# input-output-hk/plutus-halo2-verifier-gen

Measured on AMD Instinct MI355X. Metric: halo2_proofs_verified_per_sec, higher is better.
Workload: dtype u32

## Files before the change

### plutus_halo2_verifier_gen_amd/csrc/bls_consts.h

```cpp
#pragma once
#include <stdint.h>
#define H2V_DEVCONST static constexpr __device__ uint32_t
H2V_DEVCONST FP_MOD[12] = {0xffffaaabu, 0xb9feffffu, 0xb153ffffu, 0x1eabfffeu, 0xf6b0f624u, 0x6730d2a0u, 0xf38512bfu, 0x64774b84u, 0x434bacd7u, 0x4b1ba7b6u, 0x397fe69au, 0x1a0111eau};
static constexpr uint32_t FP_N0 = 0xfffcfffdu;
H2V_DEVCONST FP_ONE[12] = {0x0347fcb8u, 0x19d80000u, 0x6d2002b1u, 0x12e00cdeu, 0xa2090c72u, 0x37669f83u, 0xda0f73e0u, 0x09b09b42u, 0x8f1297bbu, 0xa7c515d9u, 0xfcfa012cu, 0x0577a659u};
H2V_DEVCONST FP_R2[12] = {0x510370edu, 0x626d1c34u, 0xc53e243du, 0xd65aec45u, 0x3317d3b1u, 0x4f36a009u, 0x5d74088bu, 0x8c10ea72u, 0x75865d11u, 0xd507320au, 0xa759fd5cu, 0x0c8d4cc8u};
H2V_DEVCONST FP_MOD28[14] = {0xfffaaabu, 0xfefffffu, 0x3ffffb9u, 0xfffeb15u, 0x6241eabu, 0xa0f6b0fu, 0xf6730d2u, 0xf38512bu, 0x4774b84u, 0x4bacd76u, 0xba7b643u, 0xe69a4b1u, 0x1ea397fu, 0x001a011u};
static constexpr uint32_t FP_N0_28 = 0xffcfffdu;
static constexpr uint32_t FP_FOLD_M = 0x9d83u;
H2V_DEVCONST FP_ONE28[14] = {0x347fcb8u, 0xd800000u, 0x2b119u, 0xcde6d2u, 0xc7212e0u, 0x83a2090u, 0x37669fu, 0xda0f73eu, 0x9b09b42u, 0x1297bb0u, 0x515d98fu, 0x12ca7cu, 0x659fcfau, 0x577au};
H2V_DEVCONST FP_C23P28[14] = {0xcda8c09u, 0x8faaaaau, 0x15720a4u, 0x893d93u, 0xfad6c24u, 0x8d68ebau, 0x54754b0u, 0x8d36a8du, 0x7f2d603u, 0xd0496f2u, 0x7467875u, 0xa2fbde3u, 0xf8a1126u, 0xc501u};
H2V_DEVCONST FP_C23N28[14] = {0x3251ea2u, 0x6f55555u, 0x2a8df15u, 0xf76ad82u, 0x676b287u, 0x138dc54u, 0xa1fdc22u, 0x664e69eu, 0xc847581u, 0x7b63683u, 0x4613dcdu, 0x439e6ceu, 0x2602859u, 0xdb0fu};
H2V_DEVCONST F28_KP[5][14] = {{0x0u, 0x0u, 0x0u, 0x0u, 0x0u, 0x0u, 0x0u, 0x0u, 0x0u, 0x0u, 0x0u, 0x0u, 0x0u, 0x0u}, {0xfffaaabu, 0xfefffffu, 0x3ffffb9u, 0xfffeb15u, 0x6241eabu, 0xa0f6b0fu, 0xf6730d2u, 0xf38512bu, 0x4774b84u, 0x4bacd76u, 0xba7b643u, 0xe69a4b1u, 0x1ea397fu, 0x1a011u}, {0xfff5556u, 0xfdfffffu, 0x7ffff73u, 0xfffd62au, 0xc483d57u, 0x41ed61eu, 0xece61a5u, 0xe70a257u, 0x8ee9709u, 0x9759aecu, 0x74f6c86u, 0xcd34963u, 0x3d472ffu, 0x34022u}, {0xfff0001u, 0xfcfffffu, 0xbffff2du, 0xfffc13fu, 0x26c5c03u, 0xe2e412eu, 0xe359277u, 0xda8f383u, 0xd65e28eu, 0xe306862u, 0x2f722c9u, 0xb3cee15u, 0x5beac7fu, 0x4e033u}, {0xffeaaacu, 0xfbfffffu, 0xffffee7u, 0xfffac54u, 0x8907aafu, 0x83dac3du, 0xd9cc34au, 0xce144afu, 0x1dd2e13u, 0x2eb35d9u, 0xe9ed90du, 0x9a692c6u, 0x7a8e5ffu, 0x68044u}};
H2V_DEVCONST F28_BIAS_3_1[14] = {0x2fff0001u, 0x2fcffffdu, 0x2bffff2bu, 0x2fffc13du, 0x226c5c01u, 0x2e2e412cu, 0x2e359275u, 0x2da8f381u, 0x2d65e28cu, 0x2e306860u, 0x22f722c7u, 0x2b3cee13u, 0x25beac7du, 0x4e031u};
H2V_DEVCONST F28_BIAS_5_2[14] = {0x3ffe5557u, 0x3faffffcu, 0x33fffe9eu, 0x3fff9767u, 0x3eb49958u, 0x324d1749u, 0x3d03f41au, 0x3c1995d8u, 0x36547995u, 0x37a6034cu, 0x3a468f4du, 0x38103775u, 0x39931f7cu, 0x82052u};
H2V_DEVCONST F28_BIAS_6_1[14] = {0x2ffe0002u, 0x2f9ffffdu, 0x27fffe59u, 0x2fff827du, 0x24d8b805u, 0x2c5c825au, 0x2c6b24edu, 0x2b51e705u, 0x2acbc51bu, 0x2c60d0c3u, 0x25ee4591u, 0x2679dc28u, 0x2b7d58fdu, 0x9c064u};
H2V_DEVCONST F28_BIAS_7_1[14] = {0x2ffdaaadu, 0x2f8ffffdu, 0x2bfffe13u, 0x2fff6d92u, 0x2afcd6b1u, 0x266bed69u, 0x2bd255c0u, 0x2a8a3831u, 0x2f4310a0u, 0x211b9e39u, 0x2195fbd5u, 0x24e380dau, 0x2d67927du, 0xb6075u};
H2V_DEVCONST F28_BIAS_9_4[14] = {0x5ffd0003u, 0x5f6ffffau, 0x53fffd84u, 0x5fff43bau, 0x57451406u, 0x5a8ac385u, 0x5aa0b762u, 0x58fada86u, 0x5831a7a7u, 0x5a913923u, 0x58e56858u, 0x51b6ca3au, 0x513c057au, 0xea095u};
H2V_DEVCONST F28_BIAS_11_1[14] = {0x2ffc5559u, 0x2f4ffffdu, 0x2bfffcfbu, 0x2fff19e7u, 0x238d5161u, 0x2ea999a7u, 0x296f190au, 0x276b7ce1u, 0x21203eb4u, 0x2406d413u, 0x2034d4e2u, 0x2e8a13a1u, 0x2510787cu, 0x11e0bau};
H2V_DEVCONST F28_BIAS_13_2[14] = {0x3ffbaaafu, 0x3f2ffffcu, 0x33fffc6eu, 0x3ffef011u, 0x3fd58eb8u, 0x32c86fc4u, 0x383d7aafu, 0x35dc1f38u, 0x3a0ed5bdu, 0x3d7c6efeu, 0x37844167u, 0x3b5d5d03u, 0x38e4eb7bu, 0x1520dbu};
H2V_DEVCONST F28_BIAS_17_8[14] = {0x9ffa555bu, 0x9eeffff6u, 0x93fffb50u, 0x9ffe9c60u, 0x98660962u, 0x9b061bfcu, 0x95da3df3u, 0x92bd63e2u, 0x9bec03cbu, 0x9067a4d1u, 0x96231a6fu, 0x9503efc4u, 0x908dd175u, 0x1ba11au};
H2V_DEVCONST F28_BIAS_20_1[14] = {0x2ff9555cu, 0x2ebffffdu, 0x2ffffa85u, 0x2ffe5da6u, 0x2ad2656du, 0x29345d31u, 0x240fd072u, 0x2066576du, 0x2951e661u, 0x2e980d3bu, 0x291a3d3fu, 0x2040dde0u, 0x264c7dfcu, 0x208154u};
H2V_DEVCONST F28_BIAS_21_1[14] = {0x2ff90007u, 0x2eaffffdu, 0x23fffa3fu, 0x2ffe48bcu, 0x20f68419u, 0x2343c841u, 0x23770145u, 0x2f9ea899u, 0x2dc931e5u, 0x2352dab1u, 0x24c1f383u, 0x2eaa8292u, 0x2836b77bu, 0x222165u};
H2V_DEVCONST F28_BIAS_29_2[14] = {0x3ff6555fu, 0x3e2ffffcu, 0x33fff80eu, 0x3ffda165u, 0x32177978u, 0x33bf20bbu, 0x3eb087d9u, 0x396131f7u, 0x31838e0cu, 0x39294663u, 0x31ffa59cu, 0x31f7a81fu, 0x3788837au, 0x2f21edu};
H2V_DEVCONST F28_BIAS_32_1[14] = {0x2ff55560u, 0x2dfffffdu, 0x2ffff73du, 0x2ffd62a5u, 0x2483d57du, 0x21ed61eau, 0x2ce61a52u, 0x270a257cu, 0x2ee9709cu, 0x2759aec6u, 0x24f6c867u, 0x2d349635u, 0x2d472ffau, 0x340221u};
H2V_DEVCONST FP_MOD30[13] = {0x3fffaaabu, 0x27fbffffu, 0x153ffffbu, 0x2affffacu, 0x30f6241eu, 0x34a83dau, 0x112bf673u, 0x12e13ce1u, 0x2cd76477u, 0x1ed90d2eu, 0x29a4b1bau, 0x3a8e5ff9u, 0x1a0111u};
static constexpr uint32_t FP_MINV30 = 0x30003u;
H2V_DEVCONST FP_R3[12] = {0xd1f7b890u, 0x22294cc4u, 0x56c9f3afu, 0xc0ccb5bau, 0xd975ccb5u, 0x89a8c5c0u, 0x6c968b4cu, 0x922672eau, 0xa691de8cu, 0x7c835652u, 0xbbb98497u, 0x141ab424u};
H2V_DEVCONST FR_MOD30[9] = {0x1u, 0x3ffffffcu, 0x3fe5bfefu, 0x2f6900bfu, 0x21d80553u, 0x27602026u, 0x17d48333u, 0x29d4ca67u, 0x73edu};
static constexpr uint32_t FR_MINV30 = 0x1u;
H2V_DEVCONST FP_B[12] = {0x0d1ff2e0u, 0x67600000u, 0xb4800ac4u, 0x4b803379u, 0x882431c8u, 0xdd9a7e0eu, 0x683dcf80u, 0x26c26d0bu, 0x3c4a5eecu, 0x9f145766u, 0xf3e804b2u, 0x15de9967u};
H2V_DEVCONST FP_TWO224[12] = {0x883cb548u, 0x5e8f53dbu, 0x0373eaf8u, 0xb9b546d2u, 0x1904502cu, 0x51b9fef6u, 0xe94c8520u, 0x8388341au, 0x58c0fea4u, 0x2865518au, 0x2cc4653du, 0x0a82ce35u};
H2V_DEVCONST FP_HALF_PLAIN[12] = {0xffffd555u, 0xdcff7fffu, 0x58a9ffffu, 0x0f55ffffu, 0x7b587b12u, 0xb3986950u, 0x79c2895fu, 0xb23ba5c2u, 0x21a5d66bu, 0x258dd3dbu, 0x1cbff34du, 0x0d0088f5u};
H2V_DEVCONST FP_SQRT_EXP[12] = {0xffffeaabu, 0xee7fbfffu, 0xac54ffffu, 0x07aaffffu, 0x3dac3d89u, 0xd9cc34a8u, 0x3ce144afu, 0xd91dd2e1u, 0x90d2eb35u, 0x92c6e9edu, 0x8e5ff9a6u, 0x0680447au};
#define FP_SQRT_CHAIN_LEN 79
static constexpr __device__ uint8_t FP_SQRT_CHAIN[79][2] = {{4, 6}, {9, 0}, {4, 0}, {7, 7}, {4, 2}, {6, 3}, {6, 5}, {4, 7}, {4, 7}, {6, 6}, {6, 6}, {6, 4}, {3, 1}, {7, 6}, {4, 6}, {6, 7}, {5, 6}, {4, 4}, {8, 6}, {6, 5}, {3, 2}, {3, 1}, {6, 6}, {4, 3}, {3, 1}, {3, 0}, {6, 3}, {4, 3}, {5, 4}, {4, 3}, {8, 4}, {3, 3}, {5, 3}, {7, 2}, {7, 4}, {5, 5}, {4, 7}, {3, 1}, {5, 3}, {4, 1}, {8, 6}, {5, 2}, {2, 0}, {9, 7}, {5, 6}, {3, 1}, {8, 7}, {3, 1}, {7, 4}, {9, 7}, {4, 2}, {5, 5}, {4, 7}, {4, 7}, {4, 7}, {3, 3}, {5, 5}, {6, 2}, {5, 4}, {4, 7}, {4, 7}, {4, 7}, {4, 7}, {4, 6}, {2, 1}, {6, 7}, {4, 7}, {5, 7}, {4, 7}, {4, 7}, {4, 7}, {4, 7}, {4, 7}, {4, 7}, {4, 7}, {3, 2}, {4, 2}, {4, 2}, {3, 1}};
H2V_DEVCONST FP_BETA[12] = {0x8a75929au, 0x9d681b79u, 0x2bf22a3eu, 0xbb45abc0u, 0xe6e7e4e5u, 0x81411755u, 0x6d04f1b4u, 0xcae3387du, 0x4b54acb0u, 0x8b50a4c7u, 0xe0665613u, 0x076f2b64u};
H2V_DEVCONST FP_BETA_GLV[12] = {0x72421b59u, 0x02bee486u, 0x1841d310u, 0x50864760u, 0x6dc004ccu, 0xae891bc7u, 0xac70ad2au, 0x8fe377c4u, 0x68e4686bu, 0x1805ed15u, 0x5c1f8f5au, 0x0d1a402bu};
H2V_DEVCONST GLV_LAMBDA[4] = {0xffffffffu, 0x00000000u, 0x0001a402u, 0xac45a401u};
H2V_DEVCONST GLV_MU[8] = {0xc4b6396eu, 0xed2f27c6u, 0x9345fbd1u, 0x1c4fa4d3u, 0x7b67f718u, 0xb1fb7291u, 0xf00fd56eu, 0xbe35f678u};
H2V_DEVCONST FR_MOD[8] = {0x00000001u, 0xffffffffu, 0xfffe5bfeu, 0x53bda402u, 0x09a1d805u, 0x3339d808u, 0x299d7d48u, 0x73eda753u};
static constexpr uint32_t FR_N0 = 0xffffffffu;
H2V_DEVCONST FR_ONE[8] = {0xfffffffeu, 0x00000001u, 0x00034802u, 0x5884b7fau, 0xecbc4ff5u, 0x998c4fefu, 0xacc5056fu, 0x1824b159u};
H2V_DEVCONST FR_R2[8] = {0xf3f29c6du, 0xc999e990u, 0x87925c23u, 0x2b6cedcbu, 0x7254398fu, 0x05d31496u, 0x9f59ff11u, 0x0748d9d9u};
H2V_DEVCONST FR_R3[8] = {0x439b73afu, 0xc62c1807u, 0x8cf06990u, 0x1b3e0d18u, 0xc7b5f418u, 0x73d13c71u, 0xc8db33e9u, 0x6e2a5bb9u};
static constexpr uint64_t BLS_X_ABS = 0xd201000000010000ull;
__device__ const uint32_t FROB_GAMMA[6][2][12] = {
    {{0x0347fcb8u, 0x19d80000u, 0x6d2002b1u, 0x12e00cdeu, 0xa2090c72u, 0x37669f83u, 0xda0f73e0u, 0x09b09b42u, 0x8f1297bbu, 0xa7c515d9u, 0xfcfa012cu, 0x0577a659u}, {0x00000000u, 0x00000000u, 0x00000000u, 0x00000000u, 0x00000000u, 0x00000000u, 0x00000000u, 0x00000000u, 0x00000000u, 0x00000000u, 0x00000000u, 0x00000000u}},
    {{0x19f1ba38u, 0x18ed52b3u, 0x15a3131fu, 0xde3f9328u, 0x4a4df35bu, 0x6f74657cu, 0x266b7cccu, 0xd2acd4ffu, 0x88cae398u, 0x121243b6u, 0x376fa613u, 0x01c3e72du}, {0xe60df073u, 0xa111ad4cu, 0x9bb0ece0u, 0x406c6cd6u, 0xac6302c8u, 0xf7bc6d24u, 0xcd1995f2u, 0x91ca7685u, 0xba80c93eu, 0x390963ffu, 0x02104087u, 0x183d2abdu}},
    {{0x00000000u, 0x00000000u, 0x00000000u, 0x00000000u, 0x00000000u, 0x00000000u, 0x00000000u, 0x00000000u, 0x00000000u, 0x00000000u, 0x00000000u, 0x00000000u}, {0x72421b59u, 0x02bee486u, 0x1841d310u, 0x50864760u, 0x6dc004ccu, 0xae891bc7u, 0xac70ad2au, 0x8fe377c4u, 0x68e4686bu, 0x1805ed15u, 0x5c1f8f5au, 0x0d1a402bu}},
    {{0xa33e2f27u, 0xd232a25au, 0x49e27ca1u, 0x707ac1e0u, 0x5ca94c3fu, 0x010b7b05u, 0x3b937942u, 0x3d5a86aau, 0x44a544deu, 0xda5556a0u, 0xc5159c66u, 0x0cea338eu}, {0xa33e2f27u, 0xd232a25au, 0x49e27ca1u, 0x707ac1e0u, 0x5ca94c3fu, 0x010b7b05u, 0x3b937942u, 0x3d5a86aau, 0x44a544deu, 0xda5556a0u, 0xc5159c66u, 0x0cea338eu}},
    {{0x758a1811u, 0x1c96e486u, 0x8561d5c1u, 0x6366543eu, 0x0fc9113eu, 0xe5efbb4bu, 0x8680210au, 0x99941307u, 0xf7f70026u, 0xbfcb02eeu, 0x59199086u, 0x1291e685u}, {0x00000000u, 0x00000000u, 0x00000000u, 0x00000000u, 0x00000000u, 0x00000000u, 0x00000000u, 0x00000000u, 0x00000000u, 0x00000000u, 0x00000000u, 0x00000000u}},
    {{0xbd2fe95fu, 0xeb1ff50du, 0x5f858fc0u, 0x4eba5508u, 0xa6f73f9bu, 0x707fe081u, 0x61fef60eu, 0x10075ba9u, 0xcd702877u, 0xec679a56u, 0xfc854279u, 0x0eae1abbu}, {0x42cfc14cu, 0xcedf0af2u, 0x51ce703eu, 0xcff1aaf6u, 0x4fb9b688u, 0xf6b0f21fu, 0x91861cb0u, 0x546fefdbu, 0x75db8460u, 0x5eb40d5fu, 0x3cfaa420u, 0x0b52f72eu}},
};
H2V_DEVCONST FROB_G1_C0[12] = {0x19f1ba38u, 0x18ed52b3u, 0x15a3131fu, 0xde3f9328u, 0x4a4df35bu, 0x6f74657cu, 0x266b7cccu, 0xd2acd4ffu, 0x88cae398u, 0x121243b6u, 0x376fa613u, 0x01c3e72du};
H2V_DEVCONST FROB_G1_C1[12] = {0xe60df073u, 0xa111ad4cu, 0x9bb0ece0u, 0x406c6cd6u, 0xac6302c8u, 0xf7bc6d24u, 0xcd1995f2u, 0x91ca7685u, 0xba80c93eu, 0x390963ffu, 0x02104087u, 0x183d2abdu};
H2V_DEVCONST FROB_G2_C0[12] = {0x00000000u, 0x00000000u, 0x00000000u, 0x00000000u, 0x00000000u, 0x00000000u, 0x00000000u, 0x00000000u, 0x00000000u, 0x00000000u, 0x00000000u, 0x00000000u};
H2V_DEVCONST FROB_G2_C1[12] = {0x72421b59u, 0x02bee486u, 0x1841d310u, 0x50864760u, 0x6dc004ccu, 0xae891bc7u, 0xac70ad2au, 0x8fe377c4u, 0x68e4686bu, 0x1805ed15u, 0x5c1f8f5au, 0x0d1a402bu};
H2V_DEVCONST FROB_G3_C0[12] = {0xa33e2f27u, 0xd232a25au, 0x49e27ca1u, 0x707ac1e0u, 0x5ca94c3fu, 0x010b7b05u, 0x3b937942u, 0x3d5a86aau, 0x44a544deu, 0xda5556a0u, 0xc5159c66u, 0x0cea338eu};
H2V_DEVCONST FROB_G3_C1[12] = {0xa33e2f27u, 0xd232a25au, 0x49e27ca1u, 0x707ac1e0u, 0x5ca94c3fu, 0x010b7b05u, 0x3b937942u, 0x3d5a86aau, 0x44a544deu, 0xda5556a0u, 0xc5159c66u, 0x0cea338eu};
H2V_DEVCONST FROB_G4_C0[12] = {0x758a1811u, 0x1c96e486u, 0x8561d5c1u, 0x6366543eu, 0x0fc9113eu, 0xe5efbb4bu, 0x8680210au, 0x99941307u, 0xf7f70026u, 0xbfcb02eeu, 0x59199086u, 0x1291e685u};
H2V_DEVCONST FROB_G4_C1[12] = {0x00000000u, 0x00000000u, 0x00000000u, 0x00000000u, 0x00000000u, 0x00000000u, 0x00000000u, 0x00000000u, 0x00000000u, 0x00000000u, 0x00000000u, 0x00000000u};
H2V_DEVCONST FROB_G5_C0[12] = {0xbd2fe95fu, 0xeb1ff50du, 0x5f858fc0u, 0x4eba5508u, 0xa6f73f9bu, 0x707fe081u, 0x61fef60eu, 0x10075ba9u, 0xcd702877u, 0xec679a56u, 0xfc854279u, 0x0eae1abbu};
H2V_DEVCONST FROB_G5_C1[12] = {0x42cfc14cu, 0xcedf0af2u, 0x51ce703eu, 0xcff1aaf6u, 0x4fb9b688u, 0xf6b0f21fu, 0x91861cb0u, 0x546fefdbu, 0x75db8460u, 0x5eb40d5fu, 0x3cfaa420u, 0x0b52f72eu};
```

### plutus_halo2_verifier_gen_amd/csrc/h2v_curve28.hpp

```cpp
#pragma once
#include "h2v_curve.hpp"
#include "h2v_fp28.hpp"

struct G1J28 { F28 x, y, z; };

H2V_DI void g1j28_from_affine(G1J28 &r, const G1A &a) {
    f28_from_fp(r.x, a.x);
    f28_from_fp(r.y, a.y);
    f28_set_one(r.z);
}
H2V_DI void g1j28_to_g1j(G1J &r, const G1J28 &p, const bool inf) {
    if (inf) { g1j_set_inf(r); return; }
    F28 z = p.z;
    f28_carry(z);
    f28_to_fp(r.x, p.x);
    f28_to_fp(r.y, p.y);
    f28_to_fp(r.z, z);
}
#define F28_MUL_(r, a, b) do { if (INL) f28_mul_inl(r, a, b); else f28_mul(r, a, b); } while (0)
#define F28_SQR_(r, a) do { if (INL) f28_sqr_inl(r, a); else f28_sqr(r, a); } while (0)
template <bool INL>
H2V_DI void g1j28_dbl_t(G1J28 &r, const G1J28 &p) {
    F28 X = p.x, Y = p.y, Z = p.z, A, B, D, t;
    F28_NEG(t, Y, 21, 1);
// ... 183 lines not shown
    F28_SUB(R, S2, Y1, 21, 1);
#pragma unroll
    for (int i = 0; i < 14; i++) { x.l[i] = l == 0 ? H.l[i] : (l == 1 ? X1.l[i] : R.l[i]); y.l[i] = l == 2 ? R.l[i] : HH.l[i]; }
    f28_mul_inl(r, x, y);
    const F28 HHH = f28_bcast<0>(r), V = f28_bcast<1>(r), RR = f28_bcast<2>(r);
    F28 X3, Y3;
    F28_SUB(X3, RR, HHH, 3, 1);
    f28_mul_small<2>(t, V);
    F28_SUB(X3, X3, t, 5, 2); f28_carry(X3);
    F28_SUB(t, V, X3, 11, 1);
#pragma unroll
    for (int i = 0; i < 14; i++) { x.l[i] = l == 0 ? R.l[i] : Y1.l[i]; y.l[i] = l == 0 ? t.l[i] : HHH.l[i]; }
    f28_mul_inl(r, x, y);
    const F28 c = f28_bcast<0>(r), yh = f28_bcast<1>(r);
    F28_SUB(Y3, c, yh, 3, 1); f28_carry(Y3);
    p.x = X3; p.y = Y3; p.z = Z3;
}

template <int N>
H2V_DI void g1j28_batch_to_affine(F28 (&ax)[N], F28 (&ay)[N], const G1J28 (&pts)[N]) {
    F28 pre[N];
    pre[0] = pts[0].z;
    f28_carry(pre[0]);
#pragma unroll 1
    for (int i = 1; i < N; i++) f28_mul(pre[i], pre[i - 1], pts[i].z);
    Fp pc, ic;
    f28_to_fp(pc, pre[N - 1]);
    (void)fp_inv(ic, pc);
    F28 inv;
    f28_from_fp(inv, ic);
#pragma unroll 1
    for (int i = N - 1; i >= 0; i--) {
        F28 zi, z2, t;
        if (i > 0) { f28_mul(zi, inv, pre[i - 1]); f28_mul(t, inv, pts[i].z); inv = t; } else zi = inv;
        f28_sqr(z2, zi);
        f28_mul(ax[i], pts[i].x, z2);
        f28_mul(z2, z2, zi);
        f28_mul(ay[i], pts[i].y, z2);
    }
}
H2V_DN void g1j28_dbl_ool(G1J28 &r, const G1J28 &p) { g1j28_dbl(r, p); }
H2V_DN int g1j28_add_ool(G1J28 &r, const G1J28 &p, const G1J28 &q) { return g1j28_add(r, p, q, false); }
H2V_DI void g1_store_table_entry(uint32_t *dst, const F28 &x, const F28 &y) {
    uint4 *q = reinterpret_cast<uint4 *>(dst);
    q[0] = make_uint4(x.l[0], x.l[1], x.l[2], x.l[3]);
    q[1] = make_uint4(x.l[4], x.l[5], x.l[6], x.l[7]);
    q[2] = make_uint4(x.l[8], x.l[9], x.l[10], x.l[11]);
    q[3] = make_uint4(x.l[12], x.l[13], y.l[0], y.l[1]);
    q[4] = make_uint4(y.l[2], y.l[3], y.l[4], y.l[5]);
    q[5] = make_uint4(y.l[6], y.l[7], y.l[8], y.l[9]);
    q[6] = make_uint4(y.l[10], y.l[11], y.l[12], y.l[13]);
}
template <int N>
H2V_DI void g1j28_table_to_affine(uint32_t *tab , const G1J28 (&pts)[N]) {
    F28 run = pts[0].z;
    f28_carry(run);
#pragma unroll 1
    for (int i = 1; i < N; i++) {
        uint4 *q = reinterpret_cast<uint4 *>(tab + i * 28);
        q[0] = make_uint4(run.l[0], run.l[1], run.l[2], run.l[3]); q[1] = make_uint4(run.l[4], run.l[5], run.l[6], run.l[7]);
        q[2] = make_uint4(run.l[8], run.l[9], run.l[10], run.l[11]); q[3] = make_uint4(run.l[12], run.l[13], 0u, 0u);
        f28_mul(run, run, pts[i].z);
    }
    Fp pc, ic;
    f28_to_fp(pc, run);
    (void)fp_inv(ic, pc);
    F28 inv;
    f28_from_fp(inv, ic);
#pragma unroll 1
    for (int i = N - 1; i >= 0; i--) {
        F28 zi, z2, t, x, y;
        if (i > 0) {
            const uint4 *q = reinterpret_cast<const uint4 *>(tab + i * 28);
            const uint4 a = q[0], b = q[1], c = q[2], d = q[3];
            F28 pre;
            pre.l[0] = a.x; pre.l[1] = a.y; pre.l[2] = a.z; pre.l[3] = a.w; pre.l[4] = b.x; pre.l[5] = b.y; pre.l[6] = b.z; pre.l[7] = b.w;
            pre.l[8] = c.x; pre.l[9] = c.y; pre.l[10] = c.z; pre.l[11] = c.w; pre.l[12] = d.x; pre.l[13] = d.y;
            f28_mul(zi, inv, pre);
            f28_mul(t, inv, pts[i].z);
            inv = t;
        } else {
            zi = inv;
        }
        f28_sqr(z2, zi);
        f28_mul(x, pts[i].x, z2);
        f28_mul(z2, z2, zi);
        f28_mul(y, pts[i].y, z2);
        g1_store_table_entry(tab + (i + 1) * 28, x, y);
    }
}
H2V_DN void g1_build_window_table(uint32_t *tab, const G1A &base) {
    G1J28 t1, e[7];
    g1j28_from_affine(t1, base);
    g1j28_dbl(e[0], t1);
    g1j28_madd_ladder(e[1], e[0], t1.x, t1.y, false);
    g1j28_dbl(e[2], e[0]);
    g1j28_madd_ladder(e[3], e[2], t1.x, t1.y, false);
    g1j28_dbl(e[4], e[1]);
    g1j28_madd_ladder(e[5], e[4], t1.x, t1.y, false);
    g1j28_dbl(e[6], e[2]);
    g1_store_table_entry(tab, t1.x, t1.y);
    g1j28_table_to_affine<7>(tab, e);
}
H2V_DN void g1_build_window_tables_glv(uint32_t *tab2, const G1A &base) {
    g1_build_window_table(tab2, base);
    Fp beta;
#pragma unroll
    for (int k = 0; k < 12; k++) beta.v[k] = FP_BETA_GLV[k];
    F28 b28;
    f28_from_fp(b28, beta);
#pragma unroll 1
    for (int m = 0; m < 8; m++) {
        F28 x, y, bx;
#pragma unroll
        for (int k = 0; k < 14; k++) { x.l[k] = tab2[m * 28 + k]; y.l[k] = tab2[m * 28 + 14 + k]; }
        f28_mul(bx, x, b28);
        g1_store_table_entry(tab2 + 224 + m * 28, bx, y);
    }
}
H2V_DI void g1j28_acc_add(G1J28 &acc, bool &acc_inf, const G1J28 &q, const bool neg) {
    if (acc_inf) {
        acc = q;
        if (neg) { F28 ny; F28_NEG(ny, q.y, 20, 1); f28_carry(ny); acc.y = ny; }
        acc_inf = false;
        return;
    }
    const int k = g1j28_add(acc, acc, q, neg);
    if (k == 2) acc_inf = true;
}

template <bool AFFINE>
H2V_DN void g1j28_mul_x_abs(G1J28 &r, bool &r_inf, const G1J28 &p, const bool p_inf) {
    G1J28 acc = p;
    bool inf = p_inf;
    F28 zz, zzz;
    f28_set_zero(zz);
    f28_set_zero(zzz);
    if (!AFFINE && !p_inf) {
        f28_sqr(zz, p.z);
        f28_mul(zzz, p.z, zz);
    }
#pragma unroll 1
    for (int i = 62; i >= 0; i--) {
        if (!inf) g1j28_dbl_t<true>(acc, acc);
        if (((BLS_X_ABS >> i) & 1) && !p_inf) {
            if (inf) {
                acc = p;
                inf = false;
            } else {
                const int k = AFFINE ? g1j28_madd_complete(acc, acc, p.x, p.y) : g1j28_add_zz(acc, acc, p, false, zz, zzz);
                if (k == 2) inf = true;
            }
        }
    }
    r = acc;
    r_inf = inf;
}
H2V_DN bool g1a_in_subgroup28(const G1A &a) {
    G1J28 p, t;
    bool tinf = false;
    g1j28_from_affine(p, a);
    g1j28_mul_x_abs<true>(t, tinf, p, false);
    g1j28_mul_x_abs<false>(t, tinf, t, tinf);
    if (tinf) return false;
    G1J tj;
    g1j28_to_g1j(tj, t, false);
    Fp beta, z2, z3, l, ny;
#pragma unroll
    for (int i = 0; i < 12; i++) beta.v[i] = FP_BETA[i];
    fp_sqr(z2, tj.z);
    fp_mul(z3, z2, tj.z);
// ... 7 lines not shown
```

### plutus_halo2_verifier_gen_amd/csrc/h2v_field.hpp

```cpp
#pragma once
#include <hip/hip_runtime.h>
#include <stdint.h>
#include "bls_consts.h"

#define H2V_DI __device__ __forceinline__
#define H2V_DN __device__ __noinline__

template <int N>
struct Big {
    uint32_t v[N];
};
using Fp = Big<12>;
using Fr = Big<8>;

struct FpParams {
    static constexpr int N = 12;
    H2V_DI static uint32_t mod(int i) { return FP_MOD[i]; }
    H2V_DI static uint32_t one(int i) { return FP_ONE[i]; }
    H2V_DI static uint32_t r2(int i) { return FP_R2[i]; }
    static constexpr uint32_t n0 = FP_N0;
};
struct FrParams {
    static constexpr int N = 8;
    H2V_DI static uint32_t mod(int i) { return FR_MOD[i]; }
// ... 339 lines not shown
    return r;
}
H2V_DI void fr_mul(Fr &r, const Fr &a, const Fr &b) {
    const FrRegs z = fr_mul_raw(u32x4{a.v[0], a.v[1], a.v[2], a.v[3]}, u32x4{a.v[4], a.v[5], a.v[6], a.v[7]},
                                u32x4{b.v[0], b.v[1], b.v[2], b.v[3]}, u32x4{b.v[4], b.v[5], b.v[6], b.v[7]});
    r.v[0] = z.a.x; r.v[1] = z.a.y; r.v[2] = z.a.z; r.v[3] = z.a.w; r.v[4] = z.b.x; r.v[5] = z.b.y; r.v[6] = z.b.z; r.v[7] = z.b.w;
}
H2V_DI void fr_to_mont(Fr &r, const Fr &plain) {
    Fr k;
#pragma unroll
    for (int i = 0; i < 8; i++) k.v[i] = FR_R2[i];
    fr_mul(r, plain, k);
}
H2V_DI void fr_from_mont(Fr &r, const Fr &a) {
    Fr one;
#pragma unroll
    for (int i = 0; i < 8; i++) one.v[i] = i == 0 ? 1u : 0u;
    fr_mul(r, a, one);
}
H2V_DI void fr_add(Fr &r, const Fr &a, const Fr &b) { FrF::add(r, a, b); }
H2V_DI void fr_sub(Fr &r, const Fr &a, const Fr &b) { FrF::sub(r, a, b); }

H2V_DI void fp_to_mont(Fp &r, const Fp &plain) {
    Fp k;
#pragma unroll
    for (int i = 0; i < 12; i++) k.v[i] = FP_R2[i];
    fp_mul(r, plain, k);
}
H2V_DI void fp_from_mont(Fp &r, const Fp &a) {
    Fp one;
    fp_set_zero(one);
    one.v[0] = 1;
    fp_mul(r, a, one);
}
#include "h2v_modinv.hpp"
H2V_DN bool fp_inv(Fp &r, const Fp &a) {
    if (fp_is_zero(a)) { fp_set_zero(r); return false; }
    Fp x, c;
    ModInv30<13>::inverse<12>(x.v, a.v, FP_MOD30, FP_MINV30);
#pragma unroll
    for (int i = 0; i < 12; i++) c.v[i] = FP_R3[i];
    fp_mul(r, x, c);
    return true;
}
H2V_DN bool fr_inv(Fr &r, const Fr &a) {
    if (FrF::is_zero(a)) { FrF::set_zero(r); return false; }
    Fr x, c;
    ModInv30<9>::inverse<8>(x.v, a.v, FR_MOD30, FR_MINV30);
#pragma unroll
    for (int i = 0; i < 8; i++) c.v[i] = FR_R3[i];
    fr_mul(r, x, c);
    return true;
}
H2V_DI bool fp_is_lex_larger(const Fp &a_mont) {
    Fp a;
    fp_from_mont(a, a_mont);
    uint64_t br = 0;
#pragma unroll
    for (int i = 0; i < 12; i++) {
        uint64_t d = (uint64_t)FP_HALF_PLAIN[i] - a.v[i] - br;
        br = (d >> 63) & 1;
    }
    return br != 0;
}
```

### plutus_halo2_verifier_gen_amd/csrc/h2v_fp28.hpp

```cpp
#pragma once
#include "h2v_field.hpp"

struct F28 { uint32_t l[14]; };
typedef uint32_t u32x2 __attribute__((ext_vector_type(2)));
struct F28Regs { u32x4 a, b, c; u32x2 d; };

H2V_DI F28Regs f28_pack(const F28 &x) {
    F28Regs r;
    r.a = u32x4{x.l[0], x.l[1], x.l[2], x.l[3]};
    r.b = u32x4{x.l[4], x.l[5], x.l[6], x.l[7]};
    r.c = u32x4{x.l[8], x.l[9], x.l[10], x.l[11]};
    r.d = u32x2{x.l[12], x.l[13]};
    return r;
}
H2V_DI F28 f28_unpack(const u32x4 a, const u32x4 b, const u32x4 c, const u32x2 d) {
    F28 x;
    x.l[0] = a.x; x.l[1] = a.y; x.l[2] = a.z; x.l[3] = a.w;
    x.l[4] = b.x; x.l[5] = b.y; x.l[6] = b.z; x.l[7] = b.w;
    x.l[8] = c.x; x.l[9] = c.y; x.l[10] = c.z; x.l[11] = c.w;
    x.l[12] = d.x; x.l[13] = d.y;
    return x;
}
H2V_DN F28Regs f28_mul_raw(u32x4 a0, u32x4 a1, u32x4 a2, u32x2 a3, u32x4 b0, u32x4 b1, u32x4 b2, u32x2 b3) {
    const F28 a = f28_unpack(a0, a1, a2, a3), b = f28_unpack(b0, b1, b2, b3);
// ... 81 lines not shown
    int64_t t = 0;
#pragma unroll
    for (int i = 0; i < 14; i++) {
        t += (int64_t)a.l[i] - (int64_t)((uint64_t)q * FP_MOD28[i]);
        a.l[i] = i < 13 ? (uint32_t)t & FP28_MASK : (uint32_t)t;
        t >>= 28;
    }
}
H2V_DI bool f28_is_zero_v5(const F28 &a) {
    uint32_t d0 = 0, d1 = 0, d2 = 0, d3 = 0, d4 = 0;
#pragma unroll
    for (int i = 0; i < 14; i++) {
        d0 |= a.l[i];
        d1 |= a.l[i] ^ F28_KP[1][i];
        d2 |= a.l[i] ^ F28_KP[2][i];
        d3 |= a.l[i] ^ F28_KP[3][i];
        d4 |= a.l[i] ^ F28_KP[4][i];
    }
    return d0 == 0 || d1 == 0 || d2 == 0 || d3 == 0 || d4 == 0;
}
H2V_DI void f28_set_one(F28 &r) {
#pragma unroll
    for (int i = 0; i < 14; i++) r.l[i] = FP_ONE28[i];
}
H2V_DI void f28_set_zero(F28 &r) {
#pragma unroll
    for (int i = 0; i < 14; i++) r.l[i] = 0;
}
H2V_DI void f28_from_fp(F28 &r, const Fp &a) { fp_to28(r.l, a); }
H2V_DI void f28_to_fp(Fp &r, const F28 &a) {
    F28 one, t;
    f28_set_one(one);
    f28_mul(t, a, one);
    uint32_t w[12];
    fp_from28(w, t.l);
    FpF::cond_sub(r, w, 0);
}
template <int NW>
H2V_DN void f28_pow_const(F28 &r, const F28 &a, const uint32_t (&e)[NW]) {
    F28 acc;
    f28_set_one(acc);
    bool started = false;
#pragma unroll 1
    for (int i = NW * 32 - 1; i >= 0; i--) {
        if (started) f28_sqr_inl(acc, acc);
        if ((e[i >> 5] >> (i & 31)) & 1) {
            if (started) f28_mul_inl(acc, acc, a);
            else { acc = a; started = true; }
        }
    }
    r = acc;
}

H2V_DN void f28_sqrt_chain(F28 &r, const F28 &a) {
    F28 t0 = a, t1, t2, t3, t4, t5, t6, t7, a2;
    f28_sqr(a2, a);
    f28_mul(t1, t0, a2); f28_mul(t2, t1, a2); f28_mul(t3, t2, a2); f28_mul(t4, t3, a2);
    f28_mul(t5, t4, a2); f28_mul(t6, t5, a2); f28_mul(t7, t6, a2);
#define F28_PICK(dst, idx)                                                                   \
    do {                                                                                     \
        switch (idx) {                                                                       \
        case 0: dst = t0; break; case 1: dst = t1; break; case 2: dst = t2; break; case 3: dst = t3; break; \
        case 4: dst = t4; break; case 5: dst = t5; break; case 6: dst = t6; break; default: dst = t7; break; \
        }                                                                                    \
    } while (0)
    F28 acc, op;
    F28_PICK(acc, FP_SQRT_CHAIN[0][1]);
#pragma unroll 1
    for (int k = 1; k < FP_SQRT_CHAIN_LEN; k++) {
        const int nsq = FP_SQRT_CHAIN[k][0], idx = FP_SQRT_CHAIN[k][1];
#pragma unroll 1
        for (int q = 0; q < nsq; q++) f28_sqr_inl(acc, acc);
        if (idx != 255) {
            F28_PICK(op, idx);
            f28_mul_inl(acc, acc, op);
        }
    }
#undef F28_PICK
    r = acc;
}
```

### plutus_halo2_verifier_gen_amd/csrc/h2v_kernels.hip

```cpp
#include <hip/hip_runtime.h>
#include "h2v_curve28.hpp"
#include "h2v_plan.h"
#include "h2v_tower.hpp"
#include "h2v_pairing_coop.hpp"
#include "h2v_pairing_six.hpp"

__device__ static constexpr uint64_t B2_IV[8] = {
    0x6a09e667f3bcc908ull, 0xbb67ae8584caa73bull, 0x3c6ef372fe94f82bull, 0xa54ff53a5f1d36f1ull,
    0x510e527fade682d1ull, 0x9b05688c2b3e6c1full, 0x1f83d9abfb41bd6bull, 0x5be0cd19137e2179ull};
__device__ static constexpr uint8_t B2_SIGMA[12][16] = {
    {0, 1, 2, 3, 4, 5, 6, 7, 8, 9, 10, 11, 12, 13, 14, 15}, {14, 10, 4, 8, 9, 15, 13, 6, 1, 12, 0, 2, 11, 7, 5, 3},
    {11, 8, 12, 0, 5, 2, 15, 13, 10, 14, 3, 6, 7, 1, 9, 4}, {7, 9, 3, 1, 13, 12, 11, 14, 2, 6, 5, 10, 4, 0, 15, 8},
    {9, 0, 5, 7, 2, 4, 10, 15, 14, 1, 11, 12, 6, 8, 3, 13}, {2, 12, 6, 10, 0, 11, 8, 3, 4, 13, 7, 5, 15, 14, 1, 9},
    {12, 5, 1, 15, 14, 13, 4, 10, 0, 7, 6, 3, 9, 2, 8, 11}, {13, 11, 7, 14, 12, 1, 3, 9, 5, 0, 15, 4, 8, 6, 2, 10},
    {6, 15, 14, 9, 11, 3, 0, 8, 12, 2, 13, 7, 1, 4, 10, 5}, {10, 2, 8, 4, 7, 6, 1, 5, 15, 11, 9, 14, 3, 12, 13, 0},
    {0, 1, 2, 3, 4, 5, 6, 7, 8, 9, 10, 11, 12, 13, 14, 15}, {14, 10, 4, 8, 9, 15, 13, 6, 1, 12, 0, 2, 11, 7, 5, 3}};

H2V_DI uint64_t rotr64(uint64_t x, int n) { return (x >> n) | (x << (64 - n)); }

typedef __attribute__((address_space(3))) uint32_t h2v_lds_u32;
H2V_DN void b2_compress_lds(uint64_t (&h)[8], const uint32_t *msg_generic, uint64_t t, bool last) {
    const h2v_lds_u32 *msg = (const h2v_lds_u32 *)msg_generic;
    uint64_t v[16];
#pragma unroll
// ... 386 lines not shown
                      const uint8_t *__restrict__ committed, const uint8_t *__restrict__ instances,
                      uint32_t *__restrict__ pts, uint8_t *__restrict__ valid, uint32_t *__restrict__ pt_tab ,
                      const uint32_t mode, uint8_t *__restrict__ valid_sub, const uint32_t group, const uint32_t role,
                      const uint32_t lane, uint8_t *sub_ok) {
    const uint32_t slots = H2V_SLOTS(plan);
    const uint32_t gid = group * H2V_DEC_PTS + lane;
    const bool live = gid < n * slots;
    const uint32_t gg = live ? gid : 0;
    const uint32_t i = gg / slots, j = gg - i * slots;
    bool ok = live;
    const uint8_t *src = nullptr;
    const bool is_acc = j >= plan.n_points + plan.n_ci;
    if (j < plan.n_points) {
        const uint64_t off0 = proof_off[i];
        if (proof_off[i + 1] - off0 < plan.proof_len) ok = false;
        else src = proofs + off0 + plan.points[j];
    } else if (!is_acc) {
        src = committed + (size_t)i * 48;
    }
    uint32_t w[12];
#pragma unroll
    for (int k = 0; k < 12; k++) w[k] = 0;
    Fp acc_x;
    fp_set_zero(acc_x);
    if (is_acc) {
        const uint32_t s4 = 4 * (j - plan.n_points - plan.n_ci);
        const uint8_t *ins = instances + (size_t)i * plan.n_pi * 32;
        Fp cy;
        acc_coordinate(acc_x, ins, plan.acc_idx[s4 + 0], plan.acc_idx[s4 + 1]);
        acc_coordinate(cy, ins, plan.acc_idx[s4 + 2], plan.acc_idx[s4 + 3]);
        w[11] = (4u | (fp_is_lex_larger(cy) ? 1u : 0u)) << 29;
    } else if (ok) {
#pragma unroll
        for (int k = 0; k < 12; k++) {
            const uint8_t *p = src + 44 - 4 * k;
            w[k] = ((uint32_t)p[0] << 24) | ((uint32_t)p[1] << 16) | ((uint32_t)p[2] << 8) | (uint32_t)p[3];
        }
    }
    const uint32_t flags = w[11] >> 29;
    w[11] &= 0x1fffffffu;
    G1A out;
    g1a_set_inf(out);
    ok = ok && (flags & 4) != 0;
    bool finite = false;
    if (ok && (flags & 2)) {
        uint32_t any = flags & 1;
#pragma unroll
        for (int k = 0; k < 12; k++) any |= w[k];
        ok = any == 0;
    } else if (ok) {
        ok = is_acc || !FpF::geq_mod(w);
        finite = ok;
    }
    if (finite) {
        Fp x, c, t, b4;
#pragma unroll
        for (int k = 0; k < 12; k++) { t.v[k] = w[k]; b4.v[k] = FP_B[k]; }
        fp_to_mont(x, t);
        if (is_acc) x = acc_x;
        fp_sqr(c, x); fp_mul(c, c, x); fp_add(c, c, b4);
        if (role == 0) {
            Fp y, chk;
            {
                F28 c28, y28;
                f28_from_fp(c28, c);
                f28_sqrt_chain(y28, c28);
                f28_to_fp(y, y28);
            }
            fp_sqr(chk, y);
            ok = fp_eq(chk, c);
            if (ok) {
                if (fp_is_lex_larger(y) != ((flags & 1) != 0)) fp_neg(y, y);
                out.x = x; out.y = y;
                if (pt_tab) g1_build_window_tables_glv(pt_tab + (size_t)gid * 448, out);
            }
        } else {
            ok = !fp_is_zero(c);
            if (ok) {
                G1A q;
                fp_mul(q.x, c, x);
                fp_sqr(q.y, c);
                ok = g1a_in_subgroup28(q);
            }
        }
    }
    if (mode == 2) {
        if (live) valid_sub[gid] = ok ? 1 : 0;
        return;
    }
    if (mode == 0) {
        if (role == 1) sub_ok[lane] = ok ? 1 : 0;
        __syncthreads();
    }
    if (role == 0 && live) {
        if (mode == 0) ok = ok && sub_ok[lane] != 0;
        if (!ok) g1a_set_inf(out);
#pragma unroll
        for (int k = 0; k < 12; k++) { pts[(size_t)gid * 24 + k] = out.x.v[k]; pts[(size_t)gid * 24 + 12 + k] = out.y.v[k]; }
        valid[gid] = ok ? 1 : 0;
    }
}

extern "C" __global__ void __launch_bounds__(128, 2)
k_g1_decompress(H2vDevPlan plan, uint32_t n, const uint8_t *__restrict__ proofs, const uint64_t *__restrict__ proof_off,
                const uint8_t *__restrict__ committed, const uint8_t *__restrict__ instances,
                uint32_t *__restrict__ pts, uint8_t *__restrict__ valid, uint32_t *__restrict__ pt_tab ,
                uint32_t mode, uint8_t *__restrict__ valid_sub) {
    __shared__ uint8_t sub_ok[H2V_DEC_PTS];
    const uint32_t role = mode == 0 ? threadIdx.x >> 6 : mode - 1;
    dec_group(plan, n, proofs, proof_off, committed, instances, pts, valid, pt_tab, mode, valid_sub, blockIdx.x, role, threadIdx.x & 63, sub_ok);
}
extern "C" __global__ void __launch_bounds__(256, 2)
k_g1_decompress_queue(H2vDevPlan plan, uint32_t n, const uint8_t *__restrict__ proofs, const uint64_t *__restrict__ proof_off,
                      const uint8_t *__restrict__ committed, const uint8_t *__restrict__ instances,
                      uint32_t *__restrict__ pts, uint8_t *__restrict__ valid, uint32_t *__restrict__ pt_tab,
                      uint8_t *__restrict__ valid_sub, uint32_t *__restrict__ counter, uint32_t n_groups) {
    const uint32_t lane = threadIdx.x & 63;
    for (;;) {
        uint32_t u = 0;
        if (lane == 0) u = atomicAdd(counter, 1u);
        u = __builtin_amdgcn_readfirstlane(u);
        if (u >= 2 * n_groups) break;
        if (u < n_groups) dec_group(plan, n, proofs, proof_off, committed, instances, pts, valid, pt_tab, 2u, valid_sub, u, 1u, lane, nullptr);
        else dec_group(plan, n, proofs, proof_off, committed, instances, pts, valid, pt_tab, 1u, valid_sub, u - n_groups, 0u, lane, nullptr);
    }
}

#include "h2v_msm.hpp"

H2V_DI void load_line(Fp2 &lam, Fp2 &c, const uint32_t *tab, int idx) {
    const uint32_t *p = tab + (size_t)idx * 48;
#pragma unroll
    for (int k = 0; k < 12; k++) { lam.c0.v[k] = p[k]; lam.c1.v[k] = p[12 + k]; c.c0.v[k] = p[24 + k]; c.c1.v[k] = p[36 + k]; }
}
H2V_DN void miller_loop(Fp12 &f, const G1A &p1, const uint32_t *lines1, bool skip1, const G1A &p2, const uint32_t *lines2, bool skip2) {
    fp12_set_one(f);
// ... 468 lines not shown
```

Baseline: 1.439 million.

## Fuse point decompression sqrt with window-table batch inversion via shared rsqrt

Replaces the separate square-root chain and the later batch inversion for the GLV window table with a single inverse-square-root exponentiation. The table is built on an isomorphic point (c·x, c²), and the product of its Jacobian z values is folded into the rsqrt input, so the root and the table inverse both come from one chain, removing a full Fp inversion per point. The rsqrt addition chain is also shortened by using a precomputed run element t8, and more of the work stays in the 28-bit limb representation. This adds complexity and a warp-level fallback path for when the z product is zero.

```diff
diff --git a/plutus_halo2_verifier_gen_amd/csrc/bls_consts.h b/plutus_halo2_verifier_gen_amd/csrc/bls_consts.h
--- a/plutus_halo2_verifier_gen_amd/csrc/bls_consts.h
+++ b/plutus_halo2_verifier_gen_amd/csrc/bls_consts.h
@@ -33,8 +33,11 @@
 H2V_DEVCONST FP_TWO224[12] = {0x883cb548u, 0x5e8f53dbu, 0x0373eaf8u, 0xb9b546d2u, 0x1904502cu, 0x51b9fef6u, 0xe94c8520u, 0x8388341au, 0x58c0fea4u, 0x2865518au, 0x2cc4653du, 0x0a82ce35u};
 H2V_DEVCONST FP_HALF_PLAIN[12] = {0xffffd555u, 0xdcff7fffu, 0x58a9ffffu, 0x0f55ffffu, 0x7b587b12u, 0xb3986950u, 0x79c2895fu, 0xb23ba5c2u, 0x21a5d66bu, 0x258dd3dbu, 0x1cbff34du, 0x0d0088f5u};
 H2V_DEVCONST FP_SQRT_EXP[12] = {0xffffeaabu, 0xee7fbfffu, 0xac54ffffu, 0x07aaffffu, 0x3dac3d89u, 0xd9cc34a8u, 0x3ce144afu, 0xd91dd2e1u, 0x90d2eb35u, 0x92c6e9edu, 0x8e5ff9a6u, 0x0680447au};
-#define FP_SQRT_CHAIN_LEN 79
-static constexpr __device__ uint8_t FP_SQRT_CHAIN[79][2] = {{4, 6}, {9, 0}, {4, 0}, {7, 7}, {4, 2}, {6, 3}, {6, 5}, {4, 7}, {4, 7}, {6, 6}, {6, 6}, {6, 4}, {3, 1}, {7, 6}, {4, 6}, {6, 7}, {5, 6}, {4, 4}, {8, 6}, {6, 5}, {3, 2}, {3, 1}, {6, 6}, {4, 3}, {3, 1}, {3, 0}, {6, 3}, {4, 3}, {5, 4}, {4, 3}, {8, 4}, {3, 3}, {5, 3}, {7, 2}, {7, 4}, {5, 5}, {4, 7}, {3, 1}, {5, 3}, {4, 1}, {8, 6}, {5, 2}, {2, 0}, {9, 7}, {5, 6}, {3, 1}, {8, 7}, {3, 1}, {7, 4}, {9, 7}, {4, 2}, {5, 5}, {4, 7}, {4, 7}, {4, 7}, {3, 3}, {5, 5}, {6, 2}, {5, 4}, {4, 7}, {4, 7}, {4, 7}, {4, 7}, {4, 6}, {2, 1}, {6, 7}, {4, 7}, {5, 7}, {4, 7}, {4, 7}, {4, 7}, {4, 7}, {4, 7}, {4, 7}, {4, 7}, {3, 2}, {4, 2}, {4, 2}, {3, 1}};
+#define FP_RSQRT_CHAIN_LEN 71
+#define FP_RSQRT_CHAIN_RUN 8
+#define FP_RSQRT_RUN_BUILD_LEN 1
+static constexpr __device__ uint8_t FP_RSQRT_RUN_BUILD[1][2] = {{4, 7}};
+static constexpr __device__ uint8_t FP_RSQRT_CHAIN[71][2] = {{4, 6}, {9, 0}, {4, 0}, {7, 7}, {4, 2}, {6, 3}, {6, 5}, {8, 8}, {6, 6}, {6, 6}, {6, 4}, {3, 1}, {7, 6}, {4, 6}, {6, 7}, {5, 6}, {4, 4}, {8, 6}, {6, 5}, {3, 2}, {3, 1}, {6, 6}, {4, 3}, {3, 1}, {3, 0}, {6, 3}, {4, 3}, {5, 4}, {4, 3}, {8, 4}, {3, 3}, {5, 3}, {7, 2}, {7, 4}, {5, 5}, {4, 7}, {3, 1}, {5, 3}, {4, 1}, {8, 6}, {5, 2}, {2, 0}, {9, 7}, {5, 6}, {3, 1}, {8, 7}, {3, 1}, {7, 4}, {9, 7}, {4, 2}, {5, 5}, {8, 8}, {4, 7}, {3, 3}, {5, 5}, {6, 2}, {5, 4}, {8, 8}, {8, 8}, {4, 6}, {2, 1}, {10, 8}, {9, 8}, {8, 8}, {8, 8}, {8, 8}, {3, 2}, {4, 2}, {4, 2}, {2, 0}, {1, 255}};
 H2V_DEVCONST FP_BETA[12] = {0x8a75929au, 0x9d681b79u, 0x2bf22a3eu, 0xbb45abc0u, 0xe6e7e4e5u, 0x81411755u, 0x6d04f1b4u, 0xcae3387du, 0x4b54acb0u, 0x8b50a4c7u, 0xe0665613u, 0x076f2b64u};
 H2V_DEVCONST FP_BETA_GLV[12] = {0x72421b59u, 0x02bee486u, 0x1841d310u, 0x50864760u, 0x6dc004ccu, 0xae891bc7u, 0xac70ad2au, 0x8fe377c4u, 0x68e4686bu, 0x1805ed15u, 0x5c1f8f5au, 0x0d1a402bu};
 H2V_DEVCONST GLV_LAMBDA[4] = {0xffffffffu, 0x00000000u, 0x0001a402u, 0xac45a401u};
diff --git a/plutus_halo2_verifier_gen_amd/csrc/h2v_curve28.hpp b/plutus_halo2_verifier_gen_amd/csrc/h2v_curve28.hpp
--- a/plutus_halo2_verifier_gen_amd/csrc/h2v_curve28.hpp
+++ b/plutus_halo2_verifier_gen_amd/csrc/h2v_curve28.hpp
@@ -259,7 +259,7 @@
     q[6] = make_uint4(y.l[10], y.l[11], y.l[12], y.l[13]);
 }
 template <int N>
-H2V_DI void g1j28_table_to_affine(uint32_t *tab , const G1J28 (&pts)[N]) {
+H2V_DI F28 g1j28_table_park(uint32_t *tab , const G1J28 (&pts)[N]) {
     F28 run = pts[0].z;
     f28_carry(run);
 #pragma unroll 1
@@ -269,20 +269,23 @@
         q[2] = make_uint4(run.l[8], run.l[9], run.l[10], run.l[11]); q[3] = make_uint4(run.l[12], run.l[13], 0u, 0u);
         f28_mul(run, run, pts[i].z);
     }
-    Fp pc, ic;
-    f28_to_fp(pc, run);
-    (void)fp_inv(ic, pc);
-    F28 inv;
-    f28_from_fp(inv, ic);
+    return run;
+}
+template <int N>
+H2V_DI void g1j28_table_backsub(uint32_t *tab, const G1J28 (&pts)[N], F28 inv, const F28 *kept = nullptr) {
 #pragma unroll 1
     for (int i = N - 1; i >= 0; i--) {
         F28 zi, z2, t, x, y;
         if (i > 0) {
-            const uint4 *q = reinterpret_cast<const uint4 *>(tab + i * 28);
-            const uint4 a = q[0], b = q[1], c = q[2], d = q[3];
             F28 pre;
-            pre.l[0] = a.x; pre.l[1] = a.y; pre.l[2] = a.z; pre.l[3] = a.w; pre.l[4] = b.x; pre.l[5] = b.y; pre.l[6] = b.z; pre.l[7] = b.w;
-            pre.l[8] = c.x; pre.l[9] = c.y; pre.l[10] = c.z; pre.l[11] = c.w; pre.l[12] = d.x; pre.l[13] = d.y;
+            if (kept) {
+                pre = kept[i - 1];
+            } else {
+                const uint4 *q = reinterpret_cast<const uint4 *>(tab + i * 28);
+                const uint4 a = q[0], b = q[1], c = q[2], d = q[3];
+                pre.l[0] = a.x; pre.l[1] = a.y; pre.l[2] = a.z; pre.l[3] = a.w; pre.l[4] = b.x; pre.l[5] = b.y; pre.l[6] = b.z; pre.l[7] = b.w;
+                pre.l[8] = c.x; pre.l[9] = c.y; pre.l[10] = c.z; pre.l[11] = c.w; pre.l[12] = d.x; pre.l[13] = d.y;
+            }
             f28_mul(zi, inv, pre);
             f28_mul(t, inv, pts[i].z);
             inv = t;
@@ -296,9 +299,17 @@
         g1_store_table_entry(tab + (i + 1) * 28, x, y);
     }
 }
-H2V_DN void g1_build_window_table(uint32_t *tab, const G1A &base) {
-    G1J28 t1, e[7];
-    g1j28_from_affine(t1, base);
+template <int N>
+H2V_DI void g1j28_table_to_affine(uint32_t *tab, const G1J28 (&pts)[N]) {
+    const F28 run = g1j28_table_park<N>(tab, pts);
+    Fp pc, ic;
+    f28_to_fp(pc, run);
+    (void)fp_inv(ic, pc);
+    F28 inv;
+    f28_from_fp(inv, ic);
+    g1j28_table_backsub<N>(tab, pts, inv);
+}
+H2V_DI void g1j28_window_multiples(G1J28 (&e)[7], const G1J28 &t1 ) {
     g1j28_dbl(e[0], t1);
     g1j28_madd_ladder(e[1], e[0], t1.x, t1.y, false);
     g1j28_dbl(e[2], e[0]);
@@ -306,11 +317,15 @@
     g1j28_dbl(e[4], e[1]);
     g1j28_madd_ladder(e[5], e[4], t1.x, t1.y, false);
     g1j28_dbl(e[6], e[2]);
+}
+H2V_DN void g1_build_window_table(uint32_t *tab, const G1A &base) {
+    G1J28 t1, e[7];
+    g1j28_from_affine(t1, base);
+    g1j28_window_multiples(e, t1);
     g1_store_table_entry(tab, t1.x, t1.y);
     g1j28_table_to_affine<7>(tab, e);
 }
-H2V_DN void g1_build_window_tables_glv(uint32_t *tab2, const G1A &base) {
-    g1_build_window_table(tab2, base);
+H2V_DI void g1_store_glv_table(uint32_t *tab2) {
     Fp beta;
 #pragma unroll
     for (int k = 0; k < 12; k++) beta.v[k] = FP_BETA_GLV[k];
@@ -324,6 +339,83 @@
         f28_mul(bx, x, b28);
         g1_store_table_entry(tab2 + 224 + m * 28, bx, y);
     }
+}
+H2V_DN void g1_build_window_tables_glv(uint32_t *tab2, const G1A &base) {
+    g1_build_window_table(tab2, base);
+    g1_store_glv_table(tab2);
+}
+template <bool TABLES>
+H2V_DN bool g1_root_unit(Fp &y_out, uint32_t *tab2 , const F28 &x, const bool want_larger) {
+    F28 c, t;
+    {
+        Fp b4;
+#pragma unroll
+        for (int k = 0; k < 12; k++) b4.v[k] = FP_B[k];
+        F28 b28, one;
+        f28_from_fp(b28, b4);
+        f28_set_one(one);
+        f28_sqr(t, x);
+        f28_dot2(c, t, x, b28, one);
+    }
+    G1J28 e[7];
+    F28 pre[6];
+    F28 u, ev = c;
+    bool u0 = false;
+    if (TABLES) {
+        G1J28 p1;
+        f28_mul(p1.x, c, x);
+        f28_sqr(p1.y, c);
+        f28_set_one(p1.z);
+        g1j28_window_multiples(e, p1);
+        u = e[0].z;
+        f28_carry(u);
+#pragma unroll 1
+        for (int i = 1; i < 7; i++) {
+            pre[i - 1] = u;
+            f28_mul(u, u, e[i].z);
+        }
+        u0 = f28_is_zero_v5(u);
+        f28_sqr(t, u);
+        f28_sqr(t, t);
+        f28_mul(ev, c, t);
+    }
+    F28 v, w, y;
+    f28_rsqrt_chain(v, ev);
+    if (TABLES) {
+        f28_mul(w, v, u);
+        f28_mul(t, w, u);
+        f28_mul(y, c, t);
+        if (__any(u0 ? 1 : 0)) {
+            f28_rsqrt_chain(v, c);
+            f28_mul(t, c, v);
+            if (u0) y = t;
+        }
+    } else {
+        w = v;
+        f28_mul(y, c, v);
+    }
+    f28_sqr(t, y);
+    F28_SUB(t, t, c, 3, 1); f28_carry(t);
+    if (!f28_is_zero_v5(t)) return false;
+    F28 plain_one;
+    f28_set_zero(plain_one);
+    plain_one.l[0] = 1;
+    f28_mul(t, y, plain_one);
+    Fp yp, yc;
+    f28_to_fp_v2(yp, t);
+    f28_to_fp_v2(yc, y);
+    const bool flip = fp_plain_is_lex_larger(yp) != want_larger;
+    if (flip) fp_neg(yc, yc);
+    y_out = yc;
+    if (TABLES && !u0) {
+        if (flip) { F28_NEG(t, w, 3, 1); f28_carry(t); w = t; }
+        F28 y1;
+        f28_from_fp(y1, yc);
+        g1_store_table_entry(tab2, x, y1);
+        g1j28_table_backsub<7>(tab2, e, w, pre);
+        g1_store_glv_table(tab2);
+    }
+    return true;
 }
 H2V_DI void g1j28_acc_add(G1J28 &acc, bool &acc_inf, const G1J28 &q, const bool neg) {
     if (acc_inf) {
diff --git a/plutus_halo2_verifier_gen_amd/csrc/h2v_field.hpp b/plutus_halo2_verifier_gen_amd/csrc/h2v_field.hpp
--- a/plutus_halo2_verifier_gen_amd/csrc/h2v_field.hpp
+++ b/plutus_halo2_verifier_gen_amd/csrc/h2v_field.hpp
@@ -415,14 +415,17 @@
     fr_mul(r, x, c);
     return true;
 }
+H2V_DI bool fp_plain_is_lex_larger(const Fp &a ) {
+    uint64_t br = 0;
+#pragma unroll
+    for (int i = 0; i < 12; i++) {
+        uint64_t d = (uint64_t)FP_HALF_PLAIN[i] - a.v[i] - br;
+        br = (d >> 63) & 1;
+    }
+    return br != 0;
+}
 H2V_DI bool fp_is_lex_larger(const Fp &a_mont) {
     Fp a;
     fp_from_mont(a, a_mont);
-    uint64_t br = 0;
-#pragma unroll
-    for (int i = 0; i < 12; i++) {
-        uint64_t d = (uint64_t)FP_HALF_PLAIN[i] - a.v[i] - br;
-        br = (d >> 63) & 1;
-    }
-    return br != 0;
-}
+    return fp_plain_is_lex_larger(a);
+}
diff --git a/plutus_halo2_verifier_gen_amd/csrc/h2v_fp28.hpp b/plutus_halo2_verifier_gen_amd/csrc/h2v_fp28.hpp
--- a/plutus_halo2_verifier_gen_amd/csrc/h2v_fp28.hpp
+++ b/plutus_halo2_verifier_gen_amd/csrc/h2v_fp28.hpp
@@ -157,23 +157,45 @@
     r = acc;
 }
 
-H2V_DN void f28_sqrt_chain(F28 &r, const F28 &a) {
+H2V_DI void f28_to_fp_v2(Fp &r, const F28 &a) {
+    uint32_t w[12];
+    fp_from28(w, a.l);
+    FpF::cond_sub(r, w, 0);
+}
+
+H2V_DN void f28_rsqrt_chain(F28 &r, const F28 &a) {
     F28 t0 = a, t1, t2, t3, t4, t5, t6, t7, a2;
     f28_sqr(a2, a);
     f28_mul(t1, t0, a2); f28_mul(t2, t1, a2); f28_mul(t3, t2, a2); f28_mul(t4, t3, a2);
     f28_mul(t5, t4, a2); f28_mul(t6, t5, a2); f28_mul(t7, t6, a2);
+#if FP_RSQRT_CHAIN_RUN
+    F28 t8 = t7;
+#define F28_PICK8(dst) case 8: dst = t8; break;
+#else
+#define F28_PICK8(dst)
+#endif
 #define F28_PICK(dst, idx)                                                                   \
     do {                                                                                     \
         switch (idx) {                                                                       \
         case 0: dst = t0; break; case 1: dst = t1; break; case 2: dst = t2; break; case 3: dst = t3; break; \
-        case 4: dst = t4; break; case 5: dst = t5; break; case 6: dst = t6; break; default: dst = t7; break; \
+        case 4: dst = t4; break; case 5: dst = t5; break; case 6: dst = t6; break; F28_PICK8(dst) default: dst = t7; break; \
         }                                                                                    \
     } while (0)
     F28 acc, op;
-    F28_PICK(acc, FP_SQRT_CHAIN[0][1]);
-#pragma unroll 1
-    for (int k = 1; k < FP_SQRT_CHAIN_LEN; k++) {
-        const int nsq = FP_SQRT_CHAIN[k][0], idx = FP_SQRT_CHAIN[k][1];
+#if FP_RSQRT_CHAIN_RUN
+#pragma unroll 1
+    for (int k = 0; k < FP_RSQRT_RUN_BUILD_LEN; k++) {
+        const int nsq = FP_RSQRT_RUN_BUILD[k][0], idx = FP_RSQRT_RUN_BUILD[k][1];
+#pragma unroll 1
+        for (int q = 0; q < nsq; q++) f28_sqr(t8, t8);
+        F28_PICK(op, idx);
+        f28_mul(t8, t8, op);
+    }
+#endif
+    F28_PICK(acc, FP_RSQRT_CHAIN[0][1]);
+#pragma unroll 1
+    for (int k = 1; k < FP_RSQRT_CHAIN_LEN; k++) {
+        const int nsq = FP_RSQRT_CHAIN[k][0], idx = FP_RSQRT_CHAIN[k][1];
 #pragma unroll 1
         for (int q = 0; q < nsq; q++) f28_sqr_inl(acc, acc);
         if (idx != 255) {
@@ -182,5 +204,6 @@
         }
     }
 #undef F28_PICK
+#undef F28_PICK8
     r = acc;
 }
diff --git a/plutus_halo2_verifier_gen_amd/csrc/h2v_kernels.hip b/plutus_halo2_verifier_gen_amd/csrc/h2v_kernels.hip
--- a/plutus_halo2_verifier_gen_amd/csrc/h2v_kernels.hip
+++ b/plutus_halo2_verifier_gen_amd/csrc/h2v_kernels.hip
@@ -462,36 +462,33 @@
         ok = is_acc || !FpF::geq_mod(w);
         finite = ok;
     }
-    if (finite) {
+    if (finite && role == 0) {
+        Fp t, r2;
+#pragma unroll
+        for (int k = 0; k < 12; k++) { t.v[k] = w[k]; r2.v[k] = FP_R2[k]; }
+        F28 xp, r28, x28, xa;
+        f28_from_fp(xp, t);
+        f28_from_fp(r28, r2);
+        f28_mul(x28, xp, r28);
+        f28_from_fp(xa, acc_x);
+        if (is_acc) x28 = xa;
+        Fp y;
+        const bool larger = (flags & 1) != 0;
+        ok = pt_tab ? g1_root_unit<true>(y, pt_tab + (size_t)gid * 448, x28, larger) : g1_root_unit<false>(y, nullptr, x28, larger);
+        if (ok) { f28_to_fp_v2(out.x, x28); out.y = y; }
+    } else if (finite) {
         Fp x, c, t, b4;
 #pragma unroll
         for (int k = 0; k < 12; k++) { t.v[k] = w[k]; b4.v[k] = FP_B[k]; }
         fp_to_mont(x, t);
         if (is_acc) x = acc_x;
         fp_sqr(c, x); fp_mul(c, c, x); fp_add(c, c, b4);
-        if (role == 0) {
-            Fp y, chk;
-            {
-                F28 c28, y28;
-                f28_from_fp(c28, c);
-                f28_sqrt_chain(y28, c28);
-                f28_to_fp(y, y28);
-            }
-            fp_sqr(chk, y);
-            ok = fp_eq(chk, c);
-            if (ok) {
-                if (fp_is_lex_larger(y) != ((flags & 1) != 0)) fp_neg(y, y);
-                out.x = x; out.y = y;
-                if (pt_tab) g1_build_window_tables_glv(pt_tab + (size_t)gid * 448, out);
-            }
-        } else {
-            ok = !fp_is_zero(c);
-            if (ok) {
-                G1A q;
-                fp_mul(q.x, c, x);
-                fp_sqr(q.y, c);
-                ok = g1a_in_subgroup28(q);
-            }
+        ok = !fp_is_zero(c);
+        if (ok) {
+            G1A q;
+            fp_mul(q.x, c, x);
+            fp_sqr(q.y, c);
+            ok = g1a_in_subgroup28(q);
         }
     }
     if (mode == 2) {
```

After: 1.449 million, median of 6. About the same (+0.7%).
